# dusk-network/jubjub-schnorr

Hardware: AMD Instinct MI355X
Metric: Schnorr verifications/sec (higher is better)
Workload: dtype u32 limbs (29-bit), u64 accumulators

## Files before the change

jubjub_schnorr_amd/csrc/ed29.h:

```cpp
#pragma once
#include "fq29.h"

namespace jjs {

using fe_t = fe<1, 5>;

struct ext_pt {
    fe_n x, y, z, t;
};
struct niels_pt {
    fe_t ypx, ymx, z, t2d;
};

JJS_HD fe_n fe_n_one() { return fq_as<1, 2>(fq_one()); }
JJS_HD fe_n fe_n_zero() { return fq_as<1, 2>(fq_zero()); }

JJS_HD ext_pt ext_identity() {
    ext_pt p;
    p.x = fe_n_zero(); p.y = fe_n_one(); p.z = fe_n_one(); p.t = fe_n_zero();
    return p;
}
JJS_HD ext_pt ext_from_affine(const fe_n& u, const fe_n& v) {
    ext_pt p;
    p.x = u; p.y = v; p.z = fe_n_one(); p.t = fq_mul(u, v);
    return p;
}
JJS_HD niels_pt niels_identity() {
    niels_pt n;
    n.ypx = fq_as<1, 5>(fq_one()); n.ymx = n.ypx; n.z = n.ypx; n.t2d = fq_as<1, 5>(fq_zero());
    return n;
}
JJS_HD niels_pt to_niels(const ext_pt& p) {
    niels_pt n;
    n.ypx = fq_as<1, 5>(fq_norm(fq_add(p.y, p.x)));
    n.ymx = fq_norm(fq_sub(p.y, p.x));
    n.z = fq_as<1, 5>(p.z);
    n.t2d = fq_as<1, 5>(fq_mul(p.t, fe_from_const<1, 1>(JJS_D2)));
    return n;
}
JJS_HD niels_pt niels_select(bool c, const niels_pt& a, const niels_pt& b) {
    niels_pt r;
    r.ypx = fq_select(c, a.ypx, b.ypx); r.ymx = fq_select(c, a.ymx, b.ymx);
    r.z = fq_select(c, a.z, b.z); r.t2d = fq_select(c, a.t2d, b.t2d);
    return r;
}

JJS_HD ext_pt ext_double(const ext_pt& p, bool need_t) {
    auto e = fq_dbl(fq_mul_hot(p.x, p.y));
    fe_n xx = fq_sqr_hot(p.x);
    fe_n yy = fq_sqr_hot(p.y);
    auto c2 = fq_dbl(fq_sqr_hot(p.z));
    auto g = fq_norm(fq_add(yy, xx));
    auto h = fq_sub(yy, xx);
    auto f = fq_norm(fq_sub(fq_add(c2, xx), yy));
    ext_pt r;
    r.x = fq_mul_hot(e, f);
    r.z = fq_mul_hot(f, h);
    r.y = fq_mul_hot(h, g);
    if (need_t) r.t = fq_mul_hot(g, e); else r.t = fe_n_zero();
    return r;
}

JJS_HD ext_pt ext_add_niels(const ext_pt& p, const niels_pt& n, bool neg, bool need_t) {
    fe_t n_ymx = fq_select(neg, n.ypx, n.ymx);
    fe_t n_ypx = fq_select(neg, n.ymx, n.ypx);
    auto n_t2d = fq_select(neg, fq_neg(n.t2d), fq_as<2, 6>(n.t2d));
    fe_n a = fq_mul_hot(fq_sub(p.y, p.x), n_ymx);
    fe_n b = fq_mul_hot(fq_add(p.y, p.x), n_ypx);
    fe_n c = fq_mul_hot(p.t, n_t2d);
    auto d = fq_dbl(fq_mul_hot(p.z, n.z));
    auto e = fq_sub(b, a);
    auto f = fq_norm(fq_sub(d, c));
    auto g = fq_add(d, c);
    auto h = fq_norm(fq_add(b, a));
    ext_pt r;
    r.x = fq_mul_hot(e, f);
    r.z = fq_mul_hot(f, g);
    r.y = fq_mul_hot(g, h);
    if (need_t) r.t = fq_mul_hot(h, e); else r.t = fe_n_zero();
    return r;
}
JJS_HD ext_pt ext_add_affine_niels(const ext_pt& p, const fe_t& n_ypx, const fe_t& n_ymx, const fe_t& n_t2d,
                                   bool need_t) {
    fe_n a = fq_mul_hot(fq_sub(p.y, p.x), n_ymx);
    fe_n b = fq_mul_hot(fq_add(p.y, p.x), n_ypx);
    fe_n c = fq_mul_hot(p.t, n_t2d);
    auto d = fq_dbl(p.z);
    auto e = fq_sub(b, a);
    auto f = fq_norm(fq_sub(d, c));
    auto g = fq_add(d, c);
    auto h = fq_norm(fq_add(b, a));
    ext_pt r;
    r.x = fq_mul_hot(e, f);
    r.z = fq_mul_hot(f, g);
    r.y = fq_mul_hot(g, h);
    if (need_t) r.t = fq_mul_hot(h, e); else r.t = fe_n_zero();
    return r;
}

JJS_HD bool ext_is_identity(const ext_pt& p) { return fq_is_zero(p.x) && fq_eq(p.y, p.z); }

JJS_HD bool affine_on_curve(const fe_n& u, const fe_n& v) {
    fe_n u2 = fq_sqr(u), v2 = fq_sqr(v);
    auto lhs = fq_sub(v2, u2);
    auto rhs = fq_norm(fq_add(fq_mul(fq_mul(u2, v2), fe_from_const<1, 1>(JJS_D)), fq_one()));
    return fq_eq(lhs, rhs);
}
JJS_HD bool affine_is_identity(const fe_n& u, const fe_n& v) { return fq_is_zero(u) && fq_eq(v, fq_one()); }

JJS_HD bool ext_eq_affine(const ext_pt& p, const fe_n& u, const fe_n& v) {
    return fq_eq(p.x, fq_mul(u, p.z)) && fq_eq(p.y, fq_mul(v, p.z));
}

}
```

jubjub_schnorr_amd/csrc/hades29.h:

```cpp
#pragma once
#include "fq29.h"

namespace jjs {

struct hades_state {
    fe_n s[5];
};

template <int A>
JJS_HD fe_n sbox5(const fe<2, A>& x) {
    fe_n x2 = fq_sqr_plus_const(x);
    fe_n x4 = fq_sqr(x2);
    return fq_mul(x4, x);
}

JJS_HD void hades_matrix(hades_state& o, const fe_n (&t)[5]) {
#if defined(__HIP_DEVICE_COMPILE__)
    const uint32_t* h = JJS_HS_HANKEL;
    asm(JJS_HADES_MATRIX_ASM : JJS_HADES_MATRIX_OUTPUTS : JJS_HADES_MATRIX_INPUTS : JJS_HADES_MATRIX_CLOBBERS);
#else
#pragma unroll
    for (int i = 0; i < 5; ++i) o.s[i] = fq_lincomb_small<5>(JJS_HS_MAT[i], t);
#endif
}

#if defined(__HIP_DEVICE_COMPILE__)
__device__ __forceinline__ void hades_gather5(fe_n (&out)[5], const fe_n& mine, int base) {
#pragma unroll
    for (int i = 0; i < 5; ++i) {
#pragma unroll
        for (int w = 0; w < 9; ++w) out[i].l[w] = (uint32_t)__shfl((int)mine.l[w], base + i);
    }
}
#endif
JJS_HD void hades_permute(hades_state& st, int coop = -1) {
#if defined(__HIP_DEVICE_COMPILE__)
    const int cj = coop < 4 ? coop : 4, cbase = (int)(__lane_id() & ~7u);
    uint32_t crow[5] = {0, 0, 0, 0, 0};
    if (coop >= 0) {
#pragma unroll
        for (int k = 0; k < 5; ++k) crow[k] = JJS_HS_HANKEL[cj + k];
    }
#endif
    for (int r = 0; r < 68; ++r) {
        fe_n t[5];
        if (r < 4 || r >= 64) {
            const int fr = r < 4 ? r : r - 60;
#if defined(__HIP_DEVICE_COMPILE__)
            if (coop >= 0) {
                fe_n x = st.s[4];
                fe_c rc = fe_from_const<1, 1>(JJS_HS_RC_FULL[fr][4]);
#pragma unroll
                for (int i = 3; i >= 0; --i) {
                    x = fq_select(cj == i, st.s[i], x);
                    rc = fq_select(cj == i, fe_from_const<1, 1>(JJS_HS_RC_FULL[fr][i]), rc);
                }
                const auto xc = fq_add(x, rc);
                hades_gather5(t, fq_mul_chain(fq_sqr_chain(fq_sqr_chain(xc)), xc), cbase);
                hades_gather5(st.s, fq_lincomb_small<5>(crow, t), cbase);
                continue;
            }
#endif
#pragma unroll
            for (int i = 0; i < 5; ++i) t[i] = sbox5(fq_add(st.s[i], fe_from_const<1, 1>(JJS_HS_RC_FULL[fr][i])));
        } else {
            const int k = r - 4;
#pragma unroll
            for (int i = 0; i < 4; ++i) t[i] = st.s[i];
#if defined(__HIP_DEVICE_COMPILE__)
            if (coop >= 0) {
                const auto x = fq_add(st.s[4], fe_from_const<1, 1>(JJS_HS_KAPPA[k]));
                const fe_n p = fq_mul_chain(x, fq_select(coop >= 5, fq_as<2, 3>(fe_from_const<1, 1>(JJS_HS_MU[k])), x));
                fe_n y;
#pragma unroll
                for (int w = 0; w < 9; ++w) y.l[w] = (uint32_t)__shfl((int)p.l[w], cbase + 5);
                t[4] = fq_mul_chain(fq_sqr_chain(p), y);
                hades_gather5(st.s, fq_lincomb_small<5>(crow, t), cbase);
                continue;
            }
#endif
            t[4] = fq_mul(sbox5(fq_add(st.s[4], fe_from_const<1, 1>(JJS_HS_KAPPA[k]))), fe_from_const<1, 1>(JJS_HS_MU[k]));
        }
        hades_matrix(st, t);
    }
#pragma unroll
    for (int i = 0; i < 5; ++i) st.s[i] = fq_mul(st.s[i], fe_from_const<1, 1>(JJS_HS_LAMBDA_END));
}

template <typename Fetch>
JJS_HD fe_n poseidon_digest_tagged(int n_inputs, const fe_n& tag, Fetch fetch, int coop = -1) {
    hades_state st;
    st.s[0] = tag;
#pragma unroll
    for (int i = 1; i < 5; ++i) st.s[i] = fq_as<1, 2>(fq_zero());
    const int n_blocks = (n_inputs + 3) >> 2;
    for (int blk = 0; blk < n_blocks; ++blk) {
#pragma unroll
        for (int k = 0; k < 4; ++k) {
            int e = 4 * blk + k;
            if (e < n_inputs) st.s[1 + k] = fq_reduce(fq_norm(fq_add(st.s[1 + k], fetch(e))));
        }
        hades_permute(st, coop);
    }
    return st.s[1];
}

template <typename Fetch>
JJS_HD fe_n poseidon_digest(int n_inputs, Fetch fetch, int coop = -1) {
    return poseidon_digest_tagged(n_inputs, fq_as<1, 2>(fe_from_const<1, 1>(JJS_SPONGE_TAG[n_inputs])), fetch, coop);
}

JJS_HD words8 truncate250(const fe_n& digest) {
    words8 c = fq_to_words(digest);
    c.w[7] &= 0x03ffffffu;
    return c;
}

}
```

jubjub_schnorr_amd/csrc/key_tables.h:

```cpp
#pragma once
#include "verify_core.h"
#include "decode.h"
#include "ed29_quad.h"

namespace jjs {

constexpr int KT_WINDOW_NARROW = 5, KT_WINDOW_WIDE = 6;
constexpr uint32_t KT_WIDE_MULTIPLICITY = 128;
JJS_HD constexpr int kt_positions(int w) { return (252 + w) / w; }
JJS_HD constexpr int kt_entries(int w) { return (1 << (w - 1)) + 1; }
JJS_HD constexpr int kt_table_words(int w) { return kt_entries(w) * ENTRY_WORDS; }
constexpr int KT_MAX_POSITIONS = kt_positions(KT_WINDOW_NARROW);
static_assert(KT_WINDOW_NARROW >= 4 && KT_WINDOW_WIDE <= 6 && KT_WINDOW_NARROW < KT_WINDOW_WIDE, "digit extraction assumes a digit spans at most two words");
constexpr uint32_t KT_MIN_MULTIPLICITY = 16;
constexpr uint32_t KT_MAX_PROBES = 128;
constexpr uint32_t KT_KEY_MALFORMED = 1, KT_KEY_VALID = 2;
constexpr int KT_BASE_WORDS = 36;
JJS_HD constexpr size_t kt_max(size_t a, size_t b) { return a > b ? a : b; }
JJS_HD constexpr size_t kt_base_words_for_keys(size_t narrow, size_t wide) {
    return kt_max(narrow * kt_positions(KT_WINDOW_NARROW), wide * kt_positions(KT_WINDOW_WIDE)) * KT_BASE_WORDS;
}
JJS_HD constexpr size_t kt_table_words_for_keys(size_t narrow, size_t wide) {
    return kt_max(narrow * kt_positions(KT_WINDOW_NARROW) * kt_table_words(KT_WINDOW_NARROW),
                  wide * kt_positions(KT_WINDOW_WIDE) * kt_table_words(KT_WINDOW_WIDE));
}
JJS_HD constexpr size_t kt_key_bytes(int w) { return (size_t)kt_positions(w) * (KT_BASE_WORDS + kt_table_words(w)) * 4; }

struct key_column {
    fe_src src;
    uint32_t* hash;
    uint32_t hash_mask;
    uint32_t key_bytes;
    uint32_t* rep;
    uint32_t* keyid;
    uint32_t* key_item;
    uint8_t* key_flags;
    uint8_t* key_undecodable;
    uint32_t* valid_ids;
    uint32_t* bases;
    uint32_t* tables;
    uint32_t* pool_of;
};
constexpr uint32_t KT_MEMO_NONE = 0xffffffffu;
struct key_memo {
    unsigned long long* hash;
    uint32_t hash_mask;
    uint32_t cap;
    uint32_t* key;
    uint8_t* flags;
    uint32_t* stamp;
    uint32_t* todo;
    uint32_t* hit;
    uint32_t* hdr;
};
enum : uint32_t { KT_MEMO_LIVE = 0, KT_MEMO_FLUSH = 1, KT_MEMO_OFF = 2 };
struct key_params {
    uint32_t n_cols;
    uint32_t max_keys;
    uint32_t max_keys_wide;
    uint32_t quad_chains;
    uint64_t seed;
    key_column col[2];
    uint32_t* counters;
    key_memo memo[2];
    uint64_t memo_seed;
    uint32_t memo_call;
    uint32_t memo_mode;
    uint32_t pool_cap;
    uint32_t force_window;
    uint32_t keep_order;
    uint64_t n;
    uint32_t* order;
    uint32_t* key_cursor;
};

JJS_HD key_column kt_col(const key_params& K, int32_t idx) {
    const key_column &a = K.col[0], &b = K.col[1];
    const bool z = idx == 0;
    key_column c;
    c.src.base = z ? a.src.base : b.src.base; c.src.stride = z ? a.src.stride : b.src.stride; c.src.off = z ? a.src.off : b.src.off;
    c.hash = z ? a.hash : b.hash; c.hash_mask = z ? a.hash_mask : b.hash_mask; c.key_bytes = z ? a.key_bytes : b.key_bytes;
    c.rep = z ? a.rep : b.rep; c.keyid = z ? a.keyid : b.keyid; c.key_item = z ? a.key_item : b.key_item;
    c.key_flags = z ? a.key_flags : b.key_flags; c.key_undecodable = z ? a.key_undecodable : b.key_undecodable; c.bases = z ? a.bases : b.bases; c.tables = z ? a.tables : b.tables;
    c.valid_ids = z ? a.valid_ids : b.valid_ids; c.pool_of = z ? a.pool_of : b.pool_of;
    return c;
}
JJS_HD key_memo kt_memo(const key_params& K, int32_t idx) {
    const key_memo &a = K.memo[0], &b = K.memo[1];
    const bool z = idx == 0;
    key_memo m;
    m.hash = z ? a.hash : b.hash; m.hash_mask = z ? a.hash_mask : b.hash_mask; m.cap = z ? a.cap : b.cap; m.key = z ? a.key : b.key;
    m.flags = z ? a.flags : b.flags; m.stamp = z ? a.stamp : b.stamp; m.todo = z ? a.todo : b.todo; m.hit = z ? a.hit : b.hit;
    m.hdr = z ? a.hdr : b.hdr;
    return m;
}

JJS_HD uint64_t kt_hash(const fe_src& src, uint64_t item, uint32_t bytes, uint64_t seed) {
    uint64_t h = 0x9e3779b97f4a7c15ull ^ seed;
#pragma unroll
    for (uint32_t off = 0; off < 64; off += 32) {
        if (off >= bytes) break;
        const words8 w = load_words(src, item, off);
#pragma unroll
        for (int i = 0; i < 8; i += 2) {
            h ^= ((uint64_t)w.w[i + 1] << 32) | w.w[i];
            h *= 0xff51afd7ed558ccdull;
            h ^= h >> 29;
        }
    }
    return h;
}
JJS_HD bool kt_same_key(const fe_src& src, uint64_t a, uint64_t b, uint32_t bytes) {
    uint32_t diff = 0;
#pragma unroll
    for (uint32_t off = 0; off < 64; off += 32) {
        if (off >= bytes) break;
        const words8 x = load_words(src, a, off), y = load_words(src, b, off);
#pragma unroll
        for (int i = 0; i < 8; ++i) diff |= x.w[i] ^ y.w[i];
    }
    return diff == 0;
}

JJS_HD uint32_t kt_pool(const key_column& C, uint32_t id) { return C.pool_of ? C.pool_of[id] : id; }
JJS_HD uint32_t* kt_base(const key_column& C, uint32_t p, uint32_t pos, int w) {
    return C.bases + ((size_t)p * kt_positions(w) + pos) * KT_BASE_WORDS;
}
JJS_HD uint32_t* kt_table(const key_column& C, uint32_t p, uint32_t pos, int w) {
    return C.tables + ((size_t)p * kt_positions(w) + pos) * kt_table_words(w);
}
JJS_HD void kt_store_ext(uint32_t* dst, const ext_pt& p) {
#pragma unroll
    for (int i = 0; i < 9; ++i) { dst[i] = p.x.l[i]; dst[9 + i] = p.y.l[i]; dst[18 + i] = p.z.l[i]; dst[27 + i] = p.t.l[i]; }
}
JJS_HD ext_pt kt_load_ext(const uint32_t* src) {
    ext_pt p;
#pragma unroll
    for (int i = 0; i < 9; ++i) { p.x.l[i] = src[i]; p.y.l[i] = src[9 + i]; p.z.l[i] = src[18 + i]; p.t.l[i] = src[27 + i]; }
    return p;
}

JJS_HD void kt_decode_key(const key_column& C, uint32_t id, uint8_t* out, const dlog_tables& T) {
    const uint64_t item = C.key_item[id];
    const decoded_point d = decompress_point(load_words(C.src, item), T);
    store_words(out, 2 * item, d.u);
    store_words(out, 2 * item + 1, d.v);
    C.key_undecodable[id] = d.ok ? 0 : 1;
}
JJS_HD void kt_unpack_item(const key_column& C, uint64_t item, uint8_t* out, uint8_t* bad) {
    const uint32_t r = C.rep[item];
    if (r != (uint32_t)item) {
        const fe_src o{out, 64, 0};
        store_words(out, 2 * item, load_words(o, r));
        store_words(out, 2 * item + 1, load_words(o, r, 32));
    }
    if (C.key_undecodable[C.keyid[item]]) bad[item] = 1;
}

JJS_HD bool kt_chain_key(const key_column& C, uint32_t id, int w) {
    const uint64_t item = C.key_item[id];
    const words8 uw = load_words(C.src, item), vw = load_words(C.src, item, 32);
    const bool canonical = words_lt(uw, JJS_Q_WORDS) && words_lt(vw, JJS_Q_WORDS);
    const fe_n pu = fq_from_words(uw), pv = fq_from_words(vw);
    const bool valid = canonical && point_on_curve_not_identity(pu, pv) && is_torsion_free(pu, pv);
    C.key_flags[id] = (uint8_t)((canonical ? 0u : KT_KEY_MALFORMED) | (valid ? KT_KEY_VALID : 0u));
    ext_pt p = ext_from_affine(pu, pv);
    const uint32_t pi = kt_pool(C, id);
    kt_store_ext(kt_base(C, pi, 0, w), p);
    const uint32_t positions = (uint32_t)kt_positions(w);
    for (uint32_t pos = 1; pos < positions; ++pos) {
#pragma unroll 1
        for (int j = 0; j < w; ++j) p = ext_double(p, j == w - 1);
        kt_store_ext(kt_base(C, pi, pos, w), p);
    }
    return valid;
}

#if defined(__HIPCC__)
__device__ __forceinline__ void kt_chain_key_quad(const key_column& C, uint32_t id, int w, uint32_t j) {
    const uint64_t item = C.key_item[id];
    const fe_n pu = fq_from_words(load_words(C.src, item)), pv = fq_from_words(load_words(C.src, item, 32));
    ext_pt p = ext_from_affine(pu, pv);
    const uint32_t pi = kt_pool(C, id);
    if (j == 0) kt_store_ext(kt_base(C, pi, 0, w), p);
    const uint32_t positions = (uint32_t)kt_positions(w);
    for (uint32_t pos = 1; pos < positions; ++pos) {
        fe_n own;
#pragma unroll 1
        for (int k = 0; k < w; ++k) p = ext_double_quad(p, j, own);
        uint32_t* dst = kt_base(C, pi, pos, w) + 9 * j;
#pragma unroll
        for (int i = 0; i < 9; ++i) dst[i] = own.l[i];
    }
}
#endif
JJS_HD bool kt_key_flags(const key_column& C, uint32_t id) {
    const uint64_t item = C.key_item[id];
    const words8 uw = load_words(C.src, item), vw = load_words(C.src, item, 32);
    const bool canonical = words_lt(uw, JJS_Q_WORDS) && words_lt(vw, JJS_Q_WORDS);
    const fe_n pu = fq_from_words(uw), pv = fq_from_words(vw);
    const bool valid = canonical && point_on_curve_not_identity(pu, pv) && is_torsion_free(pu, pv);
    C.key_flags[id] = (uint8_t)((canonical ? 0u : KT_KEY_MALFORMED) | (valid ? KT_KEY_VALID : 0u));
    return valid;
}

JJS_HD bool kt_memo_same(const key_column& C, uint64_t item, const uint32_t* mk) {
    const words8 a = load_words(C.src, item), b = load_words(C.src, item, 32);
    uint32_t diff = 0;
#pragma unroll
    for (int i = 0; i < 8; ++i) diff |= (a.w[i] ^ mk[i]) | (b.w[i] ^ mk[8 + i]);
    return diff == 0;
}
JJS_HD bool kt_memo_match(const key_column& C, const key_memo& M, uint32_t id, bool live, uint64_t seed, uint32_t call) {
    uint32_t p = KT_MEMO_NONE;
    if (live) {
        const uint64_t item = C.key_item[id];
        const unsigned long long wrote = M.hdr[1];
        uint32_t slot = (uint32_t)kt_hash(C.src, item, 64, seed) & M.hash_mask;
        for (uint32_t probe = 0; probe < KT_MAX_PROBES; ++probe) {
            const unsigned long long e = M.hash[slot];
            if ((e >> 32) != wrote || (uint32_t)e == 0u) break;
            const uint32_t q = (uint32_t)e - 1u;
            if (q < M.cap && kt_memo_same(C, item, M.key + (size_t)16 * q)) { p = q; break; }
            slot = (slot + 1u) & M.hash_mask;
        }
    }
    M.hit[id] = p;
    if (p == KT_MEMO_NONE) {
        C.pool_of[id] = id;
        return false;
    }
    C.pool_of[id] = p;
    C.key_flags[id] = M.flags[p];
    M.stamp[p] = call;
    return true;
}
JJS_HD bool kt_memo_free(const key_memo& M, uint32_t p, uint32_t call) { return M.stamp[p] != call; }
JJS_HD void kt_memo_insert(const key_column& C, const key_memo& M, uint32_t id, uint32_t p, uint64_t seed, uint32_t call) {
    const unsigned long long mine = ((unsigned long long)call << 32) | (unsigned long long)(p + 1u);
    uint32_t slot = (uint32_t)kt_hash(C.src, C.key_item[id], 64, seed) & M.hash_mask;
    for (uint32_t probe = 0; probe < KT_MAX_PROBES; ++probe) {
#if defined(__HIP_DEVICE_COMPILE__)
        unsigned long long e = __atomic_load_n(&M.hash[slot], __ATOMIC_RELAXED);
        while ((e >> 32) != call) {
            const unsigned long long seen = atomicCAS(&M.hash[slot], e, mine);
            if (seen == e) return;
            e = seen;
        }
#else
        if ((M.hash[slot] >> 32) != call) { M.hash[slot] = mine; return; }
#endif
        slot = (slot + 1u) & M.hash_mask;
    }
}
JJS_HD void kt_memo_claim(const key_column& C, const key_memo& M, uint32_t id, uint32_t p, uint64_t seed, uint32_t call) {
    const uint64_t item = C.key_item[id];
    const words8 a = load_words(C.src, item), b = load_words(C.src, item, 32);
    uint32_t* mk = M.key + (size_t)16 * p;
#pragma unroll
    for (int i = 0; i < 8; ++i) { mk[i] = a.w[i]; mk[8 + i] = b.w[i]; }
    M.flags[p] = 0;
    M.stamp[p] = call;
    C.pool_of[id] = p;
    kt_memo_insert(C, M, id, p, seed, call);
}
JJS_HD void kt_memo_flags(const key_column& C, const key_memo& M, uint32_t id) {
    if (M.flags) M.flags[kt_pool(C, id)] = C.key_flags[id];
}

JJS_HD void kt_build_table(uint32_t* tab, const ext_pt& p1, int entries) {
    const niels_pt n1 = to_niels(p1);
    store_niels(tab, niels_identity());
    store_niels(tab + ENTRY_WORDS, n1);
    ext_pt acc = ext_double(p1, true);
    store_niels(tab + 2 * ENTRY_WORDS, to_niels(acc));
    for (int j = 3; j < entries; ++j) {
        acc = ext_add_niels(acc, n1, false, true);
        store_niels(tab + j * ENTRY_WORDS, to_niels(acc));
    }
}
JJS_HD void kt_table_lane(const key_column& C, uint32_t id, uint32_t pos, int w) {
    const uint32_t pi = kt_pool(C, id);
    kt_build_table(kt_table(C, pi, pos, w), kt_load_ext(kt_base(C, pi, pos, w)), kt_entries(w));
}

JJS_HD constexpr uint32_t kt_recode_word(int w, int word) {
    uint32_t v = 0;
    for (int i = 0; i < kt_positions(w) - 1; ++i) {
        const int bit = w * i + w - 1;
        if ((bit >> 5) == word) v |= 1u << (bit & 31);
    }
    return v;
}
JJS_HD words8 kt_recode(const words8& s, int w) {
    constexpr uint32_t KN[8] = {kt_recode_word(KT_WINDOW_NARROW, 0), kt_recode_word(KT_WINDOW_NARROW, 1), kt_recode_word(KT_WINDOW_NARROW, 2),
                                kt_recode_word(KT_WINDOW_NARROW, 3), kt_recode_word(KT_WINDOW_NARROW, 4), kt_recode_word(KT_WINDOW_NARROW, 5),
                                kt_recode_word(KT_WINDOW_NARROW, 6), kt_recode_word(KT_WINDOW_NARROW, 7)};
    constexpr uint32_t KW[8] = {kt_recode_word(KT_WINDOW_WIDE, 0), kt_recode_word(KT_WINDOW_WIDE, 1), kt_recode_word(KT_WINDOW_WIDE, 2),
                                kt_recode_word(KT_WINDOW_WIDE, 3), kt_recode_word(KT_WINDOW_WIDE, 4), kt_recode_word(KT_WINDOW_WIDE, 5),
                                kt_recode_word(KT_WINDOW_WIDE, 6), kt_recode_word(KT_WINDOW_WIDE, 7)};
    const bool wide = w == KT_WINDOW_WIDE;
    words8 r;
    uint64_t carry = 0;
#pragma unroll
    for (int i = 0; i < 8; ++i) {
        const uint64_t t = (uint64_t)s.w[i] + (wide ? KW[i] : KN[i]) + carry;
        r.w[i] = (uint32_t)t;
        carry = t >> 32;
    }
    return r;
}
JJS_HD ext_pt kt_add_digit(const ext_pt& acc, const uint32_t* tab, const words8& sc, int pos, int w) {
    const int bit = w * pos, wi = bit >> 5, sh = bit & 31;
    uint32_t v = word_at(sc, wi) >> sh;
    if (sh + w > 32) v |= word_at(sc, wi + 1 > 7 ? 7 : wi + 1) << (32 - sh);
    const uint32_t raw = v & ((1u << w) - 1u);
    const bool top = pos == kt_positions(w) - 1;
    const int d = top ? (int)(word_at(sc, wi) >> sh) : (int)raw - (1 << (w - 1));
    const bool neg = d < 0;
    uint32_t idx = (uint32_t)(neg ? -d : d);
    idx = idx >= (uint32_t)kt_entries(w) ? (uint32_t)kt_entries(w) - 1u : idx;
    return ext_add_niels(acc, load_niels(tab + idx * ENTRY_WORDS), neg, true);
}
JJS_HD ext_pt kt_add_scalar(ext_pt acc, const key_column& C, uint32_t id, const words8& s, int w) {
    const words8 sc = kt_recode(s, w);
    const uint32_t pi = kt_pool(C, id);
    for (int pos = kt_positions(w) - 1; pos >= 0; --pos) acc = kt_add_digit(acc, kt_table(C, pi, (uint32_t)pos, w), sc, pos, w);
    return acc;
}

JJS_HD uint32_t kt_finish_item(const verify_params& P, const key_params& K, uint64_t item, const prep_record& r) {
    const int w = (int)*P.key_flag;
    const words8 u = load_words(P.u, item);
    bool keys_valid = true, keys_malformed = false, eq_ok = true;
    for (uint32_t e = 0; e < P.n_eq; ++e) {
        const eq_desc& E = P.eq[e];
        ext_pt acc = ext_identity();
        {
            const key_column C = kt_col(K, E.pk_col);
            const uint32_t id = C.keyid[item], f = C.key_flags[id];
            keys_valid = keys_valid && (f & KT_KEY_VALID) != 0;
            keys_malformed = keys_malformed || (f & KT_KEY_MALFORMED) != 0;
            acc = kt_add_scalar(acc, C, id, r.c, w);
        }
        if (E.comb) {
            acc = add_comb(acc, E.comb, u, JJS_SKIP(P, 16u));
        } else {
            const key_column C = kt_col(K, E.gen_col);
            const uint32_t id = C.keyid[item], f = C.key_flags[id];
            keys_valid = keys_valid && (f & KT_KEY_VALID) != 0;
            keys_malformed = keys_malformed || (f & KT_KEY_MALFORMED) != 0;
            acc = kt_add_scalar(acc, C, id, u, w);
        }
        const fe_n ru = load_fq(E.r, item), rv = load_fq(E.r, item, 32);
        eq_ok = ext_eq_affine(acc, ru, rv) && eq_ok;
    }
    if (r.malformed || keys_malformed || !words_lt(u, JJS_FR_WORDS)) return ST_MALFORMED;
    if (!r.valid || !keys_valid) return ST_INVALID_POINT;
    if (JJS_SKIP(P, 1u)) return eq_ok ? ST_OK : ST_INVALID_SIGNATURE;
    return eq_ok ? ST_OK : ST_PENDING_EQ_FAILED;
}

}
```

Measured before the change: 122.1 million.

## Normalize key tables to affine Niels and skip work in mixed additions

Key-table entries are now built in projective form and then batch-normalized to affine with a single field inversion (Montgomery's trick). Per-digit lookups then load only ypx, ymx and t2d and use the cheaper mixed affine addition, which saves one multiply and one entry load per digit. Two further changes: the challenge scalar skips the always-empty top window position when the wide window is used, and the final Poseidon permutation scales only the output lane on the non-cooperative path. The cost is a heavier table build and reliance on the challenge being at most 250 bits.

```diff
diff --git a/jubjub_schnorr_amd/csrc/ed29.h b/jubjub_schnorr_amd/csrc/ed29.h
--- a/jubjub_schnorr_amd/csrc/ed29.h
+++ b/jubjub_schnorr_amd/csrc/ed29.h
@@ -80,11 +80,14 @@
     if (need_t) r.t = fq_mul_hot(h, e); else r.t = fe_n_zero();
     return r;
 }
-JJS_HD ext_pt ext_add_affine_niels(const ext_pt& p, const fe_t& n_ypx, const fe_t& n_ymx, const fe_t& n_t2d,
-                                   bool need_t) {
-    fe_n a = fq_mul_hot(fq_sub(p.y, p.x), n_ymx);
-    fe_n b = fq_mul_hot(fq_add(p.y, p.x), n_ypx);
-    fe_n c = fq_mul_hot(p.t, n_t2d);
+JJS_HD ext_pt ext_add_affine_niels_signed(const ext_pt& p, const fe_t& n_ypx, const fe_t& n_ymx, const fe_t& n_t2d, bool neg,
+                                          bool need_t) {
+    fe_t s_ymx = fq_select(neg, n_ypx, n_ymx);
+    fe_t s_ypx = fq_select(neg, n_ymx, n_ypx);
+    auto s_t2d = fq_select(neg, fq_neg(n_t2d), fq_as<2, 6>(n_t2d));
+    fe_n a = fq_mul_hot(fq_sub(p.y, p.x), s_ymx);
+    fe_n b = fq_mul_hot(fq_add(p.y, p.x), s_ypx);
+    fe_n c = fq_mul_hot(p.t, s_t2d);
     auto d = fq_dbl(p.z);
     auto e = fq_sub(b, a);
     auto f = fq_norm(fq_sub(d, c));
@@ -96,6 +99,11 @@
     r.y = fq_mul_hot(g, h);
     if (need_t) r.t = fq_mul_hot(h, e); else r.t = fe_n_zero();
     return r;
+}
+
+JJS_HD ext_pt ext_add_affine_niels(const ext_pt& p, const fe_t& n_ypx, const fe_t& n_ymx, const fe_t& n_t2d,
+                                   bool need_t) {
+    return ext_add_affine_niels_signed(p, n_ypx, n_ymx, n_t2d, false, need_t);
 }
 
 JJS_HD bool ext_is_identity(const ext_pt& p) { return fq_is_zero(p.x) && fq_eq(p.y, p.z); }
diff --git a/jubjub_schnorr_amd/csrc/hades29.h b/jubjub_schnorr_amd/csrc/hades29.h
--- a/jubjub_schnorr_amd/csrc/hades29.h
+++ b/jubjub_schnorr_amd/csrc/hades29.h
@@ -33,7 +33,7 @@
     }
 }
 #endif
-JJS_HD void hades_permute(hades_state& st, int coop = -1) {
+JJS_HD void hades_permute(hades_state& st, int coop = -1, bool digest_only = false) {
 #if defined(__HIP_DEVICE_COMPILE__)
     const int cj = coop < 4 ? coop : 4, cbase = (int)(__lane_id() & ~7u);
     uint32_t crow[5] = {0, 0, 0, 0, 0};
@@ -83,6 +83,11 @@
         }
         hades_matrix(st, t);
     }
+    if (digest_only) {
+        st.s[1] = fq_mul(st.s[1], fe_from_const<1, 1>(JJS_HS_LAMBDA_END));
+        st.s[0] = st.s[2] = st.s[3] = st.s[4] = fq_as<1, 2>(fq_zero());
+        return;
+    }
 #pragma unroll
     for (int i = 0; i < 5; ++i) st.s[i] = fq_mul(st.s[i], fe_from_const<1, 1>(JJS_HS_LAMBDA_END));
 }
@@ -100,7 +105,7 @@
             int e = 4 * blk + k;
             if (e < n_inputs) st.s[1 + k] = fq_reduce(fq_norm(fq_add(st.s[1 + k], fetch(e))));
         }
-        hades_permute(st, coop);
+        hades_permute(st, coop, coop < 0 && blk == n_blocks - 1);
     }
     return st.s[1];
 }
diff --git a/jubjub_schnorr_amd/csrc/key_tables.h b/jubjub_schnorr_amd/csrc/key_tables.h
--- a/jubjub_schnorr_amd/csrc/key_tables.h
+++ b/jubjub_schnorr_amd/csrc/key_tables.h
@@ -268,15 +268,38 @@
     if (M.flags) M.flags[kt_pool(C, id)] = C.key_flags[id];
 }
 
+JJS_HD void kt_put_projective(uint32_t* dst, const ext_pt& p, const fe_n& prefix) {
+    niels_pt n;
+    n.ypx = fq_as<1, 5>(p.x); n.ymx = fq_as<1, 5>(p.y); n.z = fq_as<1, 5>(p.z); n.t2d = fq_as<1, 5>(prefix);
+    store_niels(dst, n);
+}
 JJS_HD void kt_build_table(uint32_t* tab, const ext_pt& p1, int entries) {
     const niels_pt n1 = to_niels(p1);
     store_niels(tab, niels_identity());
-    store_niels(tab + ENTRY_WORDS, n1);
+    fe_n run = fe_n_one();
+    kt_put_projective(tab + ENTRY_WORDS, p1, run);
+    run = p1.z;
     ext_pt acc = ext_double(p1, true);
-    store_niels(tab + 2 * ENTRY_WORDS, to_niels(acc));
-    for (int j = 3; j < entries; ++j) {
-        acc = ext_add_niels(acc, n1, false, true);
-        store_niels(tab + j * ENTRY_WORDS, to_niels(acc));
+    for (int j = 2; j < entries; ++j) {
+        if (j > 2) acc = ext_add_niels(acc, n1, false, true);
+        kt_put_projective(tab + j * ENTRY_WORDS, acc, run);
+        run = fq_mul_hot(run, acc.z);
+    }
+    fe_n inv = fq_inverse(run);
+    niels_pt e = load_niels(tab + (entries - 1) * ENTRY_WORDS);
+    for (int j = entries - 1; j >= 1; --j) {
+        niels_pt below = e;
+        if (j > 1) below = load_niels(tab + (j - 1) * ENTRY_WORDS);
+        const fe_n zi = fq_mul_hot(inv, e.t2d);
+        inv = fq_mul_hot(inv, e.z);
+        const fe_n u = fq_mul_hot(e.ypx, zi), v = fq_mul_hot(e.ymx, zi);
+        niels_pt n;
+        n.ypx = fq_as<1, 5>(fq_norm(fq_add(v, u)));
+        n.ymx = fq_norm(fq_sub(v, u));
+        n.z = fq_as<1, 5>(fq_one());
+        n.t2d = fq_as<1, 5>(fq_mul_hot(fq_mul_hot(u, v), fe_from_const<1, 1>(JJS_D2)));
+        store_niels(tab + j * ENTRY_WORDS, n);
+        e = below;
     }
 }
 JJS_HD void kt_table_lane(const key_column& C, uint32_t id, uint32_t pos, int w) {
@@ -310,6 +333,18 @@
     }
     return r;
 }
+JJS_HD void kt_load_affine(const uint32_t* src, fe_t& ypx, fe_t& ymx, fe_t& t2d) {
+    const u32x4* p = reinterpret_cast<const u32x4*>(src);
+    uint32_t w[ENTRY_WORDS];
+#pragma unroll
+    for (int i = 0; i < ENTRY_WORDS / 4; ++i) {
+        if (i == 5) continue;
+        const u32x4 v = p[i];
+        w[4 * i] = v.x; w[4 * i + 1] = v.y; w[4 * i + 2] = v.z; w[4 * i + 3] = v.w;
+    }
+#pragma unroll
+    for (int i = 0; i < 9; ++i) { ypx.l[i] = w[i]; ymx.l[i] = w[9 + i]; t2d.l[i] = w[27 + i]; }
+}
 JJS_HD ext_pt kt_add_digit(const ext_pt& acc, const uint32_t* tab, const words8& sc, int pos, int w) {
     const int bit = w * pos, wi = bit >> 5, sh = bit & 31;
     uint32_t v = word_at(sc, wi) >> sh;
@@ -320,12 +355,23 @@
     const bool neg = d < 0;
     uint32_t idx = (uint32_t)(neg ? -d : d);
     idx = idx >= (uint32_t)kt_entries(w) ? (uint32_t)kt_entries(w) - 1u : idx;
-    return ext_add_niels(acc, load_niels(tab + idx * ENTRY_WORDS), neg, true);
+    fe_t ypx, ymx, t2d;
+    kt_load_affine(tab + idx * ENTRY_WORDS, ypx, ymx, t2d);
+    return ext_add_affine_niels_signed(acc, ypx, ymx, t2d, neg, true);
 }
 JJS_HD ext_pt kt_add_scalar(ext_pt acc, const key_column& C, uint32_t id, const words8& s, int w) {
     const words8 sc = kt_recode(s, w);
     const uint32_t pi = kt_pool(C, id);
     for (int pos = kt_positions(w) - 1; pos >= 0; --pos) acc = kt_add_digit(acc, kt_table(C, pi, (uint32_t)pos, w), sc, pos, w);
+    return acc;
+}
+JJS_HD constexpr int kt_challenge_positions(int w) { return kt_positions(w) - (w == KT_WINDOW_WIDE ? 1 : 0); }
+static_assert(KT_WINDOW_WIDE * (kt_positions(KT_WINDOW_WIDE) - 1) >= 252 && KT_WINDOW_NARROW * (kt_positions(KT_WINDOW_NARROW) - 1) <= 250,
+              "which top positions a 250-bit scalar leaves empty");
+JJS_HD ext_pt kt_add_challenge(ext_pt acc, const key_column& C, uint32_t id, const words8& c, int w) {
+    const words8 sc = kt_recode(c, w);
+    const uint32_t pi = kt_pool(C, id);
+    for (int pos = kt_challenge_positions(w) - 1; pos >= 0; --pos) acc = kt_add_digit(acc, kt_table(C, pi, (uint32_t)pos, w), sc, pos, w);
     return acc;
 }
 
@@ -341,7 +387,7 @@
             const uint32_t id = C.keyid[item], f = C.key_flags[id];
             keys_valid = keys_valid && (f & KT_KEY_VALID) != 0;
             keys_malformed = keys_malformed || (f & KT_KEY_MALFORMED) != 0;
-            acc = kt_add_scalar(acc, C, id, r.c, w);
+            acc = kt_add_challenge(acc, C, id, r.c, w);
         }
         if (E.comb) {
             acc = add_comb(acc, E.comb, u, JJS_SKIP(P, 16u));
```

Result: faster. 125.5 million (median of 6 runs) (+2.9%).
